# Lumina-Group/libzkp

Hardware: NVIDIA B200
Metric: groth16_bn254_proofs_per_sec_batched (higher is better)
Workload: dtype u256 (8x32-bit Montgomery limbs, integer)

## Files before the change

libzkp_b200/csrc/engine.cu:

```cuda
#include <cuda_runtime.h>
#include <atomic>
#include <cmath>
#include <cstdio>
#include <cstdlib>
#include <mutex>
#include <string>
#include <thread>
#include <type_traits>
#include <vector>

#include "common.h"
#include "host_util.h"
#include "kernels_prove.cuh"
#include "tables.h"
#include "large.h"
#include "setup.h"
#include "verify.h"

using namespace lzkp;
using namespace lzkp::eng;

static thread_local std::string g_err;
static std::mutex g_mu;
static int g_device = -1;
// ... 47 lines not shown
        CUDA_TRY(cudaMemcpyToSymbol(c_mimc, c.data(), sizeof(Fr) * 110));
        g_mimc_uploaded |= 1ull << (dev & 63);
    }
    return LZKP_OK;
}
int current_device() { return t_device >= 0 ? t_device : g_device; }
DeviceScope::DeviceScope(int dev) : prev(t_device) {
    t_device = dev;
    cudaSetDevice(dev);
}
DeviceScope::~DeviceScope() {
    t_device = prev;
    const int back = prev >= 0 ? prev : g_device;
    if (back >= 0) cudaSetDevice(back);
}
}
}


struct MsmPlan {
    DBuf table;
    DBuf unit_dig, unit_tbl;
    DBuf items[4];
    DBuf msm_items[4];
    uint32_t n_items[4] = {0, 0, 0, 0};
    uint32_t item_len[4] = {8, 32, 128, 512};
    uint32_t n_units = 0, n_rows = 0, n_msm = 0;
    std::vector<uint32_t> msm_unit_begin;
    std::vector<uint2> msm_items_host[4];
};

struct HBuf {
    void *p = nullptr;
    size_t bytes = 0;
    int ensure(size_t n) {
        if (n <= bytes) return LZKP_OK;
        if (p) cudaFreeHost(p);
        p = nullptr;
        bytes = 0;
        cudaError_t err = cudaMallocHost(&p, n);
        if (err != cudaSuccess) { p = nullptr; cudaGetLastError(); return fail(LZKP_E_NOMEM, "cudaMallocHost failed"); }
        bytes = n;
        return LZKP_OK;
    }
    template <class T> T *as() const { return reinterpret_cast<T *>(p); }
    ~HBuf() { if (p) cudaFreeHost(p); }
};
struct Workspace {
    uint32_t chunk = 0;
    DBuf z, abc, tmp, h, dig, r, s, rs, part1, part2, res1, res2, proofs, status, a, b, commit, sets, setlen, env, envlen;
    HBuf h_proofs, h_status, h_commit, h_env, h_envlen;
    cudaEvent_t last_use = nullptr;
    ~Workspace() { if (last_use) cudaEventDestroy(last_use); }
};
static int ws_acquire(Workspace &ws, cudaStream_t st) {
    if (!ws.last_use) CUDA_TRY(cudaEventCreateWithFlags(&ws.last_use, cudaEventDisableTiming));
    else CUDA_TRY(cudaStreamWaitEvent(st, ws.last_use, 0));
    return LZKP_OK;
}
static int ws_release(Workspace &ws, cudaStream_t st) {
    CUDA_TRY(cudaEventRecord(ws.last_use, st));
    return LZKP_OK;
}

struct lzkp_pk {
    std::mutex mu;
    int device = 0;
    std::vector<lzkp_pk *> replicas;
    uint32_t n_vars = 0, n_inst = 0, n_wit = 0, n = 0, log_n = 0, m = 0;
    bool has_circuit = false;
    int kind = -1;
    uint32_t kind_param = 0;
    int c = 16;
    uint32_t W = 16, N = 32768;
    uint64_t table_bytes = 0;
    uint32_t max_chunk = 8192;
    uint32_t n_dig_rows = 0, nz = 0;
    MsmPlan g1, g2;
    MsmPlan g1_lat;
    uint32_t row_sz = 0, row_rz = 0;
    bool has_lat = false;
    ProofConsts consts;
    DBuf csr_rowptr[3], csr_col[3], csr_val[3];
    CsrDev csr[3];
    DBuf tw_fwd, tw_inv, coset_br, uncoset_br;
    NttTables ntt;
    Workspace ws[2];
    bool large = false;
    bool tiled_wm = false;
    MsmBases *L_a = nullptr, *L_b1 = nullptr, *L_b2 = nullptr, *L_l = nullptr, *L_h = nullptr;
    DBuf L_sa, L_sb, L_sl, L_sb1;
    cudaStream_t L_st[3] = {nullptr, nullptr, nullptr}, L_st_scale = nullptr;
    cudaEvent_t L_ev_in = nullptr, L_ev_done[3] = {nullptr, nullptr, nullptr}, L_ev_a = nullptr, L_ev_scale = nullptr;
    uint32_t shard_index = 0, shard_count = 1, map_ranks = 1;
    bool L_scaled = false;
    uint32_t L_lo[5] = {0, 0, 0, 0, 0}, L_cnt[5] = {0, 0, 0, 0, 0};
    cudaStream_t stream = nullptr, stream2 = nullptr;
    cudaEvent_t ev_fork = nullptr, ev_join[2] = {nullptr, nullptr};
    cudaStream_t chunk_stream(int i) const { return (i & 1) ? stream2 : stream; }
    struct Mark { int region; cudaEvent_t a, b; };
    std::vector<Mark> marks;
    double prof_ms[LZKP_PROFILE_REGIONS] = {0};
    uint64_t prof_count[LZKP_PROFILE_REGIONS] = {0};
    ~lzkp_pk() {
        for (lzkp_pk *r : replicas) { DeviceScope ds(r->device); delete r; }
        for (auto &m : marks) { cudaEventDestroy(m.a); cudaEventDestroy(m.b); }
        for (MsmBases *b : {L_a, L_b1, L_b2, L_l, L_h}) if (b) msm_bases_free(b);
        for (auto s_ : L_st) if (s_) cudaStreamDestroy(s_);
        if (L_ev_in) cudaEventDestroy(L_ev_in);
        if (L_ev_a) cudaEventDestroy(L_ev_a);
        if (L_ev_scale) cudaEventDestroy(L_ev_scale);
        if (L_st_scale) cudaStreamDestroy(L_st_scale);
        for (auto ev : L_ev_done) if (ev) cudaEventDestroy(ev);
        if (ev_fork) cudaEventDestroy(ev_fork);
        for (auto ev : ev_join) if (ev) cudaEventDestroy(ev);
        if (stream2) cudaStreamDestroy(stream2);
        if (stream) cudaStreamDestroy(stream);
    }
};

struct BaseRef { uint32_t dig_row, tbl_row; };
static int finish_plan(MsmPlan &pl, const std::vector<std::vector<BaseRef>> &msms, uint32_t W) {
    std::vector<uint32_t> ud, ut;
    pl.msm_unit_begin.clear();
    for (auto &ms : msms) {
        pl.msm_unit_begin.push_back((uint32_t)ud.size());
        for (auto &b : ms)
            for (uint32_t w = 0; w < W; w++) {
                ud.push_back(b.dig_row * W + w);
                ut.push_back(b.tbl_row * W + w);
            }
    }
    pl.msm_unit_begin.push_back((uint32_t)ud.size());
    pl.n_units = (uint32_t)ud.size();
    pl.n_msm = (uint32_t)msms.size();
    TRY(upload(pl.unit_dig, ud));
    TRY(upload(pl.unit_tbl, ut));
    for (int v = 0; v < 4; v++) {
        std::vector<uint2> items, mi;
        for (uint32_t q = 0; q < pl.n_msm; q++) {
            uint32_t first = (uint32_t)items.size();
            for (uint32_t u = pl.msm_unit_begin[q]; u < pl.msm_unit_begin[q + 1]; u += pl.item_len[v])
                items.push_back(make_uint2(u, std::min(u + pl.item_len[v], pl.msm_unit_begin[q + 1])));
            mi.push_back(make_uint2(first, (uint32_t)items.size()));
        }
        pl.n_items[v] = (uint32_t)items.size();
        pl.msm_items_host[v] = mi;
        TRY(upload(pl.items[v], items));
        TRY(upload(pl.msm_items[v], mi));
    }
    return LZKP_OK;
}

static uint32_t fit_item_len(const std::vector<std::vector<BaseRef>> &msms, uint32_t W, uint32_t resident) {
    uint32_t best = 128;
    uint64_t best_cost = UINT64_MAX;
    for (uint32_t len = 96; len <= 192; len++) {
        uint64_t items = 0, cost = 0;
        for (auto &ms : msms) items += ((uint64_t)ms.size() * W + len - 1) / len;
        for (uint64_t gx : {8u, 16u, 32u, 64u}) cost += (gx * items + resident - 1) / resident * len * (64 / gx);
        if (cost < best_cost) { best_cost = cost; best = len; }
    }
    return best;
}

static inline uint32_t window_count(int c) { return (uint32_t)((255 + c - 1) / c); }

namespace {
struct Reader {
    const uint8_t *p, *end;
    bool take(size_t n, const uint8_t **out) {
        if ((size_t)(end - p) < n) return false;
        *out = p;
        p += n;
        return true;
    }
    bool g1(host::G1Canon &o) { const uint8_t *b; return take(64, &b) && host::read_g1(b, o); }
    bool g2(host::G2Canon &o) { const uint8_t *b; return take(128, &b) && host::read_g2(b, o); }
    bool vec_g1(std::vector<host::G1Canon> &v) {
        const uint8_t *b;
        if (!take(8, &b)) return false;
        uint64_t len;
        memcpy(&len, b, 8);
        if (len > (uint64_t)(end - p) / 64) return false;
        v.resize(len);
        for (auto &x : v) if (!g1(x)) return false;
        return true;
    }
    bool vec_g2(std::vector<host::G2Canon> &v) {
        const uint8_t *b;
        if (!take(8, &b)) return false;
        uint64_t len;
        memcpy(&len, b, 8);
        if (len > (uint64_t)(end - p) / 128) return false;
        v.resize(len);
        for (auto &x : v) if (!g2(x)) return false;
        return true;
    }
};
host::G1Canon neg_canon(const host::G1Canon &p) {
    host::G1Canon r = p;
    if (!host::is_inf(p)) {
        Fq m = Fq::modulus();
        sub8(r.y.l, m.l, p.y.l);
    }
    return r;
}
}

static int pk_load_impl(const uint8_t *bytes, size_t len, int validate, const lzkp_pk_options *opt, lzkp_pk *pk) {
    static_assert(sizeof(host::G1Canon) == sizeof(G1Affine) && sizeof(host::G2Canon) == sizeof(G2Affine), "layout");
    Reader rd{bytes, bytes + len};
    host::G1Canon alpha_g1, beta_g1, delta_g1;
    host::G2Canon beta_g2, gamma_g2, delta_g2;
    std::vector<host::G1Canon> gamma_abc, a_q, b1_q, h_q, l_q;
    std::vector<host::G2Canon> b2_q;
    bool ok = rd.g1(alpha_g1) && rd.g2(beta_g2) && rd.g2(gamma_g2) && rd.g2(delta_g2) && rd.vec_g1(gamma_abc) &&
              rd.g1(beta_g1) && rd.g1(delta_g1) && rd.vec_g1(a_q) && rd.vec_g1(b1_q) && rd.vec_g2(b2_q) &&
              rd.vec_g1(h_q) && rd.vec_g1(l_q);
    if (!ok || rd.p != rd.end) return fail(LZKP_E_INVALID, "proving key: malformed ark-serialize bytes");
    const uint32_t nv = (uint32_t)a_q.size();
    if (nv < 2 || b1_q.size() != nv || b2_q.size() != nv || l_q.size() >= nv || gamma_abc.size() + l_q.size() != nv)
        return fail(LZKP_E_INVALID, "proving key: inconsistent query lengths");
    const uint32_t n = (uint32_t)h_q.size() + 1;
    if (n < 2 || (n & (n - 1))) return fail(LZKP_E_INVALID, "proving key: h_query length + 1 is not a power of two");
    pk->n_vars = nv;
    pk->n_wit = (uint32_t)l_q.size();
    pk->n_inst = nv - pk->n_wit;
    pk->n = n;
    pk->log_n = 0;
    while ((1u << pk->log_n) < n) pk->log_n++;
    pk->nz = nv - 1;
    pk->n_dig_rows = pk->nz + 3 + (n - 1);
    const uint32_t ROW_R = pk->nz, ROW_S = pk->nz + 1, ROW_RS = pk->nz + 2, ROW_H = pk->nz + 3;

    {
        size_t free_b0 = 0, total_b0 = 0;
        CUDA_TRY(cudaMemGetInfo(&free_b0, &total_b0));
        const uint64_t budget0 = opt && opt->table_budget_bytes ? opt->table_budget_bytes : (uint64_t)(free_b0 * 0.6);
        const uint64_t rows1_max = 2ull * nv + pk->n_wit + n + 2, rows2_max = (uint64_t)nv + 1;
        const uint64_t min_table = (rows1_max * 64 + rows2_max * 128) * 32 * 128;
        pk->large = pk->log_n > 16 || min_table > budget0 || getenv("LZKP_FORCE_LARGE") != nullptr;
    }
    if (pk->large) {
        CUDA_TRY(cudaStreamCreate(&pk->stream));
    CUDA_TRY(cudaStreamCreate(&pk->stream2));
    CUDA_TRY(cudaEventCreateWithFlags(&pk->ev_fork, cudaEventDisableTiming));
    for (auto &ev : pk->ev_join) CUDA_TRY(cudaEventCreateWithFlags(&ev, cudaEventDisableTiming));
        const int wb = opt && opt->window_bits ? opt->window_bits : 0;
        pk->shard_count = opt && opt->shard_count > 1 ? opt->shard_count : 1;
        pk->shard_index = pk->shard_count > 1 ? opt->shard_index : 0;
        if (pk->shard_index >= pk->shard_count) return fail(LZKP_E_INVALID, "shard_index >= shard_count");
        const uint32_t G_ = pk->shard_count;
        const uint64_t w_g2 = getenv("LZKP_SHARD_G2_WEIGHT") ? (uint64_t)atoi(getenv("LZKP_SHARD_G2_WEIGHT")) : (G_ > 2 ? 32 : 28);
        const uint64_t sizes[5] = {nv, nv, (uint64_t)pk->n_wit + 1, (uint64_t)n - 1, nv}, wts[5] = {10, 10, 10, 10, w_g2};
        const double Wh = (double)sizes[3] * wts[3];
        double Wz = 0;
        for (int q : {0, 1, 2, 4}) Wz += (double)sizes[q] * wts[q];
        const double map_frac = getenv("LZKP_SHARD_MAP_COST") ? atof(getenv("LZKP_SHARD_MAP_COST")) : (G_ > 4 ? 0.085 : 0.11);
        const double M = G_ > 1 ? map_frac * (Wz + Wh) : 0.0;
        uint32_t k = 1;
        while (k < G_ && k * ((Wz + Wh + k * M) / G_ - M) < Wh) k++;
        const double T = (Wz + Wh + k * M) / G_;
        std::vector<double> cutz(G_ + 1, 0.0), share(G_, 0.0);
        for (uint32_t i = 0; i < G_; i++) share[i] = i < k ? std::max(0.0, T - M - Wh / k) : T;
        const double piece_cost = G_ > 2 ? (getenv("LZKP_SHARD_PIECE_COST") ? atof(getenv("LZKP_SHARD_PIECE_COST")) : (G_ > 4 ? 0.25 : 0.45)) * 2.76e6 : 0.0;
        std::vector<double> adj(share);
        for (int round = 0; round < 4; round++) {
            double tot = 0;
            for (uint32_t i = 0; i < G_; i++) tot += adj[i];
            for (uint32_t i = 0; i < G_; i++) cutz[i + 1] = cutz[i] + adj[i] * Wz / tot;
            double bounds[5] = {0, 0, 0, 0, 0};
            { int j = 0; for (int q : {0, 1, 2, 4}) { bounds[j + 1] = bounds[j] + (double)sizes[q] * wts[q]; j++; } }
            if (piece_cost != 0.0)
                for (uint32_t i = 1; i < G_; i++)
                    for (int j = 1; j < 4; j++)
                        if (std::fabs(cutz[i] - bounds[j]) < 1.0e5) cutz[i] = bounds[j];
            if (round == 3 || piece_cost == 0.0) break;
            double extra_total = 0;
            std::vector<double> extra(G_, 0.0);
            for (uint32_t i = 0; i < G_; i++) {
                int pieces = 0;
                for (int j = 0; j < 4; j++)
                    if (std::min(cutz[i + 1], bounds[j + 1]) - std::max(cutz[i], bounds[j]) > 1e-6 * Wz) pieces++;
                extra[i] = piece_cost * std::max(0, pieces - 1);
                extra_total += extra[i];
            }
            for (uint32_t i = 0; i < G_; i++) adj[i] = std::max(0.0, share[i] - extra[i] + extra_total / G_);
        }
        pk->map_ranks = k;
        const uint32_t me = pk->shard_index;
        if (me < k) {
            pk->L_lo[3] = (uint32_t)(sizes[3] * me / k);
            pk->L_cnt[3] = (uint32_t)(sizes[3] * (me + 1) / k) - pk->L_lo[3];
        } else {
            pk->L_lo[3] = 0;
            pk->L_cnt[3] = 0;
        }
        double acc_w = 0;
        for (int q : {0, 1, 2, 4}) {
            auto first_at = [&](double w) -> uint64_t {
                if (w <= acc_w) return 0;
                return std::min<uint64_t>((uint64_t)std::ceil((w - acc_w) / wts[q]), sizes[q]);
            };
            uint64_t lo = first_at(cutz[me]), hi = me + 1 == G_ ? sizes[q] : first_at(cutz[me + 1]);
            pk->L_lo[q] = (uint32_t)lo;
            pk->L_cnt[q] = (uint32_t)(hi - lo);
            acc_w += (double)sizes[q] * wts[q];
        }
        auto load1 = [&](std::vector<host::G1Canon> v, size_t skip, const host::G1Canon *extra, int q, MsmBases **out) {
            v.erase(v.begin(), v.begin() + skip);
            if (extra) v.push_back(*extra);
            return msm_bases_load(1, reinterpret_cast<const uint8_t *>(v.data() + pk->L_lo[q]), pk->L_cnt[q], wb, 1, validate, out, 1);
// ... 48 lines not shown
            if (bad) return fail(LZKP_E_INVALID, "proving key: " + std::to_string(bad) + " point(s) off-curve or outside the subgroup");
        }
        TRY(d_out1.alloc(2 * sizeof(G1Affine))); TRY(d_out2.alloc(sizeof(G2Affine)));
        LAUNCH((k_affine_add<Fq>), 1, 1, 0, st, d_misc1.as<G1Affine>() + 0, d_misc1.as<G1Affine>() + 2, d_out1.as<G1Affine>() + 0, 0);
        LAUNCH((k_affine_add<Fq>), 1, 1, 0, st, d_misc1.as<G1Affine>() + 1, d_misc1.as<G1Affine>() + 3, d_out1.as<G1Affine>() + 1, 0);
        LAUNCH((k_affine_add<Fq2>), 1, 1, 0, st, d_misc2.as<G2Affine>() + 0, d_misc2.as<G2Affine>() + 1, d_out2.as<G2Affine>(), 0);
        G1Affine c1[2];
        G2Affine c2;
        CUDA_TRY(cudaMemcpyAsync(c1, d_out1.p, sizeof(c1), cudaMemcpyDeviceToHost, st));
        CUDA_TRY(cudaMemcpyAsync(&c2, d_out2.p, sizeof(c2), cudaMemcpyDeviceToHost, st));
        CUDA_TRY(cudaStreamSynchronize(st));
        pk->consts.a0 = c1[0]; pk->consts.b0 = c1[1]; pk->consts.b2 = c2;
        CUDA_TRY(cudaGetLastError());
        return LZKP_OK;
    }

    std::vector<host::G1Canon> rows1;
    std::vector<host::G2Canon> rows2;
    std::vector<std::vector<BaseRef>> msm1(5), msm2(1);
    std::vector<BaseRef> a_all, b1_all;
    auto add1 = [&](const host::G1Canon &p) { rows1.push_back(p); return (uint32_t)rows1.size() - 1; };
    auto same_point = [](const host::G1Canon &u, const host::G1Canon &v) {
        return memcmp(&u.x, &v.x, sizeof(Fq)) == 0 && memcmp(&u.y, &v.y, sizeof(Fq)) == 0;
    };
    for (uint32_t j = 1; j < nv; j++) {
        const bool has_a = !host::is_inf(a_q[j]), has_b = !host::is_inf(b1_q[j]);
        if (has_a && has_b && same_point(a_q[j], b1_q[j])) {
            const BaseRef ref{j - 1, add1(a_q[j])};
            msm1[4].push_back(ref); a_all.push_back(ref); b1_all.push_back(ref);
            continue;
        }
        if (has_a) { msm1[0].push_back({j - 1, add1(a_q[j])}); a_all.push_back(msm1[0].back()); }
        if (has_b) { msm1[1].push_back({j - 1, add1(b1_q[j])}); b1_all.push_back(msm1[1].back()); }
    }
    for (uint32_t j = 0; j < pk->n_wit; j++) if (!host::is_inf(l_q[j])) msm1[2].push_back({pk->n_inst + j - 1, add1(l_q[j])});
    for (uint32_t i = 0; i + 1 < n; i++) if (!host::is_inf(h_q[i])) msm1[3].push_back({ROW_H + i, add1(h_q[i])});
    if (!host::is_inf(delta_g1)) {
        uint32_t rd1 = add1(delta_g1), rnd1 = add1(neg_canon(delta_g1));
        msm1[0].push_back({ROW_R, rd1});
        msm1[1].push_back({ROW_S, rd1});
        msm1[2].push_back({ROW_RS, rnd1});
        a_all.push_back({ROW_R, rd1});
    }
    std::vector<std::vector<BaseRef>> msm1_lat(6);
    {
        pk->row_sz = pk->n_dig_rows;
        pk->row_rz = pk->n_dig_rows + pk->nz;
        msm1_lat[0] = a_all;
        msm1_lat[2] = msm1[2];
        msm1_lat[3] = msm1[3];
        for (auto &b : a_all) if (b.dig_row < pk->nz) msm1_lat[4].push_back({pk->row_sz + b.dig_row, b.tbl_row});
        for (auto &b : b1_all) msm1_lat[5].push_back({pk->row_rz + b.dig_row, b.tbl_row});
        auto mont = [](const host::G1Canon &c) { return G1Affine{Fq::from_canonical(c.x), Fq::from_canonical(c.y)}; };
        auto canon = [](const G1Affine &m) { host::G1Canon c; c.x = m.x.to_canonical(); c.y = m.y.to_canonical(); return c; };
        auto sum2 = [&](const host::G1Canon &u, const host::G1Canon &v) {
            G1XYZZ t = host::is_inf(u) ? G1XYZZ::inf() : G1XYZZ::from_affine(mont(u));
            if (!host::is_inf(v)) t.madd(mont(v));
            return t.is_inf() ? host::G1Canon{Fq::zero(), Fq::zero()} : canon(t.to_affine());
        };
        const host::G1Canon a0c = sum2(alpha_g1, a_q[0]), b0c = sum2(beta_g1, b1_q[0]), d2c = sum2(delta_g1, delta_g1);
        if (!host::is_inf(a0c)) msm1_lat[4].push_back({ROW_S, add1(a0c)});
        if (!host::is_inf(b0c)) msm1_lat[5].push_back({ROW_R, add1(b0c)});
        if (!host::is_inf(d2c)) msm1_lat[5].push_back({ROW_RS, add1(d2c)});
        pk->n_dig_rows += 2 * pk->nz;
        pk->has_lat = true;
    }
    for (uint32_t j = 1; j < nv; j++)
        if (!host::is_inf(b2_q[j])) { rows2.push_back(b2_q[j]); msm2[0].push_back({j - 1, (uint32_t)rows2.size() - 1}); }
    if (!host::is_inf(delta_g2)) { rows2.push_back(delta_g2); msm2[0].push_back({ROW_S, (uint32_t)rows2.size() - 1}); }
    pk->g1.n_rows = (uint32_t)rows1.size();
    pk->g2.n_rows = (uint32_t)rows2.size();

    size_t free_b = 0, total_b = 0;
    CUDA_TRY(cudaMemGetInfo(&free_b, &total_b));
    uint64_t budget = opt && opt->table_budget_bytes ? opt->table_budget_bytes : (uint64_t)(free_b * 0.6);
    int c = opt && opt->window_bits ? opt->window_bits : 0;
    if (const char *e = getenv("LZKP_WINDOW_BITS")) if (!c) c = atoi(e);
    auto bytes_for = [&](int cc) {
        uint64_t W = window_count(cc), N = 1ull << (cc - 1);
        return (rows1.size() * 64ull + rows2.size() * 128ull) * W * N;
    };
    if (c == 0) {
        c = 16;
        while (c > 8 && bytes_for(c) > budget) c--;
    }
    if (c < 8 || c > 17) return fail(LZKP_E_INVALID, "window_bits must be in [8,17]");
    if (bytes_for(c) > free_b) return fail(LZKP_E_NOMEM, "window tables do not fit in device memory");
    pk->c = c;
    pk->W = window_count(c);
    pk->N = 1u << (c - 1);
    pk->table_bytes = bytes_for(c);
    pk->max_chunk = opt && opt->max_chunk ? opt->max_chunk : 8192;
    if (pk->max_chunk > 32768) pk->max_chunk = 32768;

    CUDA_TRY(cudaStreamCreate(&pk->stream));
    CUDA_TRY(cudaStreamCreate(&pk->stream2));
    CUDA_TRY(cudaEventCreateWithFlags(&pk->ev_fork, cudaEventDisableTiming));
    for (auto &ev : pk->ev_join) CUDA_TRY(cudaEventCreateWithFlags(&ev, cudaEventDisableTiming));
    CUDA_TRY(cudaStreamCreateWithFlags(&pk->L_st[0], cudaStreamNonBlocking));
    CUDA_TRY(cudaEventCreateWithFlags(&pk->L_ev_in, cudaEventDisableTiming));
    CUDA_TRY(cudaEventCreateWithFlags(&pk->L_ev_done[0], cudaEventDisableTiming));
    cudaStream_t st = pk->stream;

    std::vector<host::G1Canon> misc1 = {alpha_g1, beta_g1, delta_g1, a_q[0], b1_q[0]};
    std::vector<host::G2Canon> misc2 = {beta_g2, gamma_g2, delta_g2, b2_q[0]};
    DBuf d_rows1, d_rows2, d_misc1, d_misc2, d_out1, d_out2;
    TRY(upload(d_rows1, rows1)); TRY(upload(d_rows2, rows2)); TRY(upload(d_misc1, misc1)); TRY(upload(d_misc2, misc2));
    auto to_mont = [&](DBuf &b, size_t n_fq) {
        if (n_fq) LAUNCH(k_fq_to_mont, (unsigned)((n_fq + 127) / 128), 128, 0, st, b.as<Fq>(), n_fq);
    };
    to_mont(d_rows1, rows1.size() * 2); to_mont(d_rows2, rows2.size() * 4);
    to_mont(d_misc1, misc1.size() * 2); to_mont(d_misc2, misc2.size() * 4);
    if (validate) {
        std::vector<host::G1Canon> all1 = gamma_abc;
        std::vector<host::G2Canon> all2;
        DBuf d_all1, d_bad;
        TRY(upload(d_all1, all1));
        to_mont(d_all1, all1.size() * 2);
        TRY(d_bad.alloc(sizeof(int)));
        CUDA_TRY(cudaMemsetAsync(d_bad.p, 0, sizeof(int), st));
        auto chk1 = [&](DBuf &b, size_t cnt) {
            if (cnt) LAUNCH(k_check_g1, (unsigned)((cnt + 63) / 64), 64, 0, st, b.as<G1Affine>(), (uint32_t)cnt, d_bad.as<int>());
        };
        auto chk2 = [&](DBuf &b, size_t cnt) {
            if (cnt) LAUNCH(k_check_g2, (unsigned)((cnt + 63) / 64), 64, 0, st, b.as<G2Affine>(), (uint32_t)cnt, d_bad.as<int>());
        };
        chk1(d_rows1, rows1.size()); chk1(d_misc1, misc1.size()); chk1(d_all1, all1.size());
        chk2(d_rows2, rows2.size()); chk2(d_misc2, misc2.size());
        int bad = 0;
        CUDA_TRY(cudaMemcpyAsync(&bad, d_bad.p, sizeof(int), cudaMemcpyDeviceToHost, st));
        CUDA_TRY(cudaStreamSynchronize(st));
        if (bad) return fail(LZKP_E_INVALID, "proving key: " + std::to_string(bad) + " point(s) off-curve or outside the subgroup");
    }
    TRY(d_out1.alloc(2 * sizeof(G1Affine))); TRY(d_out2.alloc(sizeof(G2Affine)));
    LAUNCH((k_affine_add<Fq>), 1, 1, 0, st, d_misc1.as<G1Affine>() + 0, d_misc1.as<G1Affine>() + 3, d_out1.as<G1Affine>() + 0, 0);
    LAUNCH((k_affine_add<Fq>), 1, 1, 0, st, d_misc1.as<G1Affine>() + 1, d_misc1.as<G1Affine>() + 4, d_out1.as<G1Affine>() + 1, 0);
    LAUNCH((k_affine_add<Fq2>), 1, 1, 0, st, d_misc2.as<G2Affine>() + 0, d_misc2.as<G2Affine>() + 3, d_out2.as<G2Affine>(), 0);
    G1Affine c1[2];
    G2Affine c2;
    CUDA_TRY(cudaMemcpyAsync(c1, d_out1.p, sizeof(c1), cudaMemcpyDeviceToHost, st));
    CUDA_TRY(cudaMemcpyAsync(&c2, d_out2.p, sizeof(c2), cudaMemcpyDeviceToHost, st));
    CUDA_TRY(cudaStreamSynchronize(st));
    pk->consts.a0 = c1[0]; pk->consts.b0 = c1[1]; pk->consts.b2 = c2;

    TRY(pk->g1.table.alloc((size_t)rows1.size() * pk->W * pk->N * sizeof(G1Affine)));
    TRY(pk->g2.table.alloc((size_t)rows2.size() * pk->W * pk->N * sizeof(G2Affine)));
    if (!rows1.empty())
        TRY(build_table_g1(d_rows1.p, (uint32_t)rows1.size(), c, pk->W, pk->N, pk->g1.table.p, st));
    if (!rows2.empty())
        TRY(build_table_g2(d_rows2.p, (uint32_t)rows2.size(), c, pk->W, pk->N, pk->g2.table.p, st));
    {
        uint32_t resident = 0;
        TRY(batch_msm_g1_resident(c > 16 ? 4 : 2, &resident));
        pk->g1.item_len[2] = fit_item_len(msm1, pk->W, resident);
    }
    TRY(finish_plan(pk->g1, msm1, pk->W));
    TRY(finish_plan(pk->g1_lat, msm1_lat, pk->W));
    TRY(finish_plan(pk->g2, msm2, pk->W));
    {
        const uint64_t per_proof = (uint64_t)nv * 32 + 7ull * n * 32 + (uint64_t)pk->n_dig_rows * pk->W * (c > 16 ? 4 : 2) +
                                   (uint64_t)pk->g1.n_items[2] * sizeof(G1XYZZ) + (uint64_t)pk->g2.n_items[1] * sizeof(G2XYZZ) +
                                   4 * sizeof(G1XYZZ) + sizeof(G2XYZZ) + 1024;
        size_t free_now = 0, total_now = 0;
        CUDA_TRY(cudaMemGetInfo(&free_now, &total_now));
        uint64_t fit = (uint64_t)(free_now * 0.4) / (2 * per_proof);
        fit = std::max<uint64_t>(32, fit / 32 * 32);
        if (pk->max_chunk > fit) pk->max_chunk = (uint32_t)fit;
    }
    CUDA_TRY(cudaGetLastError());
    return LZKP_OK;
}

static int circuit_install(lzkp_pk *pk, uint32_t m, uint32_t n_inst, uint32_t n_wit, const uint32_t *const rowptr[3],
                           const uint32_t *const col[3], const uint8_t *const val[3]) {
    if (n_inst != pk->n_inst || n_wit != pk->n_wit) return fail(LZKP_E_INVALID, "circuit shape does not match the proving key");
    uint64_t need = (uint64_t)m + n_inst;
    uint32_t n = 1;
    while (n < need) n <<= 1;
    if (n != pk->n) return fail(LZKP_E_INVALID, "circuit domain size does not match the proving key's h_query");
    pk->tiled_wm = pk->large || pk->log_n > 12;
    cudaStream_t st = pk->stream;
    for (int k = 0; k < 3; k++) {
        uint32_t nnz = rowptr[k][m];
        for (uint32_t i = 0; i < nnz; i++) if (col[k][i] >= pk->n_vars) return fail(LZKP_E_INVALID, "matrix column out of range");
        TRY(pk->csr_rowptr[k].alloc(sizeof(uint32_t) * (m + 1)));
        TRY(pk->csr_col[k].alloc(sizeof(uint32_t) * nnz));
        TRY(pk->csr_val[k].alloc(sizeof(Fr) * (size_t)nnz));
        CUDA_TRY(cudaMemcpy(pk->csr_rowptr[k].p, rowptr[k], sizeof(uint32_t) * (m + 1), cudaMemcpyHostToDevice));
        if (nnz) {
            CUDA_TRY(cudaMemcpy(pk->csr_col[k].p, col[k], sizeof(uint32_t) * nnz, cudaMemcpyHostToDevice));
            CUDA_TRY(cudaMemcpy(pk->csr_val[k].p, val[k], 32 * (size_t)nnz, cudaMemcpyHostToDevice));
            LAUNCH(k_to_r2_form, (nnz + 127) / 128, 128, 0, st, pk->csr_val[k].as<Fr>(), nnz);
        }
        pk->csr[k] = CsrDev{pk->csr_rowptr[k].as<uint32_t>(), pk->csr_col[k].as<uint32_t>(), pk->csr_val[k].as<Fr>()};
    }
    pk->m = m;
    Fr w, wi, g, gi;
    for (int i = 0; i < 8; i++) { w.l[i] = FrParams::ROOT28(i); wi.l[i] = FrParams::ROOT28_INV(i); g.l[i] = FrParams::GEN(i); gi.l[i] = FrParams::GEN_INV(i); }
    for (uint32_t i = pk->log_n; i < 28; i++) { w = w.sqr(); wi = wi.sqr(); }
    Fr ninv = host::fr_from_u64(n).inverse();
    Fr gn = g;
    for (uint32_t i = 0; i < pk->log_n; i++) gn = gn.sqr();
    Fr zinv = (gn - Fr::one()).inverse();
    if (pk->tiled_wm) {
        pk->ntt = NttTables{nullptr, nullptr, nullptr, nullptr, nullptr, ninv, zinv};
        CUDA_TRY(cudaStreamSynchronize(st));
        CUDA_TRY(cudaGetLastError());
        pk->has_circuit = true;
        return LZKP_OK;
    }
    TRY(pk->tw_fwd.alloc(sizeof(Fr) * (n / 2))); TRY(pk->tw_inv.alloc(sizeof(Fr) * (n / 2)));
    TRY(pk->coset_br.alloc(sizeof(Fr) * n)); TRY(pk->uncoset_br.alloc(sizeof(Fr) * n));
    LAUNCH(k_pow_table, (n / 2 + 127) / 128, 128, 0, st, pk->tw_fwd.as<Fr>(), w, Fr::one(), n / 2, 0u);
    LAUNCH(k_pow_table, (n / 2 + 127) / 128, 128, 0, st, pk->tw_inv.as<Fr>(), wi, Fr::one(), n / 2, 0u);
    LAUNCH(k_pow_table, (n + 127) / 128, 128, 0, st, pk->coset_br.as<Fr>(), g, ninv, n, pk->log_n);
    LAUNCH(k_pow_table, (n + 127) / 128, 128, 0, st, pk->uncoset_br.as<Fr>(), gi, ninv.to_canonical(), n, pk->log_n);
    pk->ntt = NttTables{pk->tw_fwd.as<Fr>(), pk->tw_inv.as<Fr>(), pk->coset_br.as<Fr>(), pk->uncoset_br.as<Fr>(), nullptr, ninv, zinv};
    size_t smem = (size_t)32 * n;
    if (smem > 48 * 1024) {
        CUDA_TRY(cudaFuncSetAttribute(k_ntt_icoset, cudaFuncAttributeMaxDynamicSharedMemorySize, (int)smem));
        CUDA_TRY(cudaFuncSetAttribute(k_ntt_final, cudaFuncAttributeMaxDynamicSharedMemorySize, (int)smem));
    }
    CUDA_TRY(cudaStreamSynchronize(st));
    CUDA_TRY(cudaGetLastError());
    pk->has_circuit = true;
    return LZKP_OK;
}

static inline int item_variant(uint32_t P) {
    return P > small_batch_limit() ? (P >= 256 ? 2 : 1) : 0;
}
static inline int fit_variant(const MsmPlan &pl, int v) {
    while (v < 3 && pl.n_items[v] > 65535u) v++;
    return v;
}
static inline uint32_t latency_limit() {
    static const uint32_t v = getenv("LZKP_LATENCY_BATCH") ? (uint32_t)atoi(getenv("LZKP_LATENCY_BATCH")) : 384u;
    return v;
}
static inline bool use_lat(const lzkp_pk *pk, uint32_t P) { return pk->has_lat && P <= latency_limit() && P <= small_batch_limit(); }
static inline int item_variant_g2(uint32_t P) {
    return P > small_batch_limit() ? 1 : 0;
}
static int ensure_workspace(lzkp_pk *pk, Workspace &ws, uint32_t P) {
    if (P <= ws.chunk) return LZKP_OK;
    size_t part1 = 0, part2 = 0;
    for (uint32_t pp : {std::min(P, small_batch_limit()), std::min(P, std::max(latency_limit(), 1u)), std::min(P, 255u), std::min(P, 2047u), P}) {
        part1 = std::max(part1, (size_t)pk->g1.n_items[fit_variant(pk->g1, item_variant(pp))] * pp);
        if (use_lat(pk, pp)) part1 = std::max(part1, (size_t)pk->g1_lat.n_items[fit_variant(pk->g1_lat, item_variant(pp))] * pp);
        part2 = std::max(part2, (size_t)pk->g2.n_items[fit_variant(pk->g2, item_variant_g2(pp))] * pp);
    }
    const size_t nv = pk->n_vars, n = pk->n;
    TRY(ws.z.ensure(P * nv * 32));
    TRY(ws.abc.ensure(3 * P * n * 32));
    TRY(ws.h.ensure(P * n * 32));
    if (pk->tiled_wm) TRY(ws.tmp.ensure(3 * P * n * 32));
    if (pk->large) {
        TRY(pk->L_sa.ensure(nv * 32)); TRY(pk->L_sb.ensure(nv * 32)); TRY(pk->L_sb1.ensure(nv * 32)); TRY(pk->L_sl.ensure(((size_t)pk->n_wit + 1) * 32));
    } else {
        TRY(ws.dig.ensure((size_t)pk->n_dig_rows * pk->W * P * (pk->c > 16 ? 4 : 2)));
    }
    TRY(ws.r.ensure(P * 32)); TRY(ws.s.ensure(P * 32)); TRY(ws.rs.ensure(P * 32));
    TRY(ws.part1.ensure(part1 * sizeof(G1XYZZ)));
    TRY(ws.part2.ensure(part2 * sizeof(G2XYZZ)));
    TRY(ws.res1.ensure((size_t)6 * P * sizeof(G1XYZZ)));
    TRY(ws.res2.ensure((size_t)P * sizeof(G2XYZZ)));
    TRY(ws.proofs.ensure((size_t)P * 256));
    TRY(ws.status.ensure((size_t)P * sizeof(int32_t)));
    TRY(ws.a.ensure(P * 8)); TRY(ws.b.ensure(P * 8)); TRY(ws.commit.ensure(P * 32));
    ws.chunk = P;
    return LZKP_OK;
}

static inline void wires_to_canonical(Fr *z, uint32_t P, uint32_t nv, uint32_t first, uint32_t count, cudaStream_t st) {
    const size_t total = (size_t)P * count;
    LAUNCH(k_wires_to_canonical, (unsigned)((total + 127) / 128), 128, 0, st, z, P, nv, first, count);
}

struct Region {
    lzkp_pk *pk;
    cudaStream_t st;
    cudaEvent_t b = nullptr;
    Region(lzkp_pk *pk_, int region, cudaStream_t st_) : pk(pk_), st(st_) {
        if (!g_profile.load(std::memory_order_relaxed) || pk->marks.size() > 65536) return;
        cudaEvent_t a;
        if (cudaEventCreate(&a) != cudaSuccess || cudaEventCreate(&b) != cudaSuccess) { b = nullptr; return; }
        cudaEventRecord(a, st);
        pk->marks.push_back({region, a, b});
    }
    ~Region() { if (b) cudaEventRecord(b, st); }
};

static int run_witness_map(lzkp_pk *pk, Workspace &ws, uint32_t P, cudaStream_t st) {
    const uint32_t n = pk->n, threads = std::max(32u, std::min(n / 2, 512u));
    const size_t smem = (size_t)32 * n;
    Region reg(pk, LZKP_REGION_WITNESS_MAP, st);
    if (pk->tiled_wm) {
        Fr *abc = ws.abc.as<Fr>(), *tmp = ws.tmp.as<Fr>(), *h = ws.h.as<Fr>();
        const size_t plane = (size_t)P * n;
        LAUNCH(k_spmv_abc, dim3((n + 127) / 128, P), 128, 0, st, pk->csr[0], pk->csr[1], pk->csr[2], ws.z.as<Fr>(), abc, P,
               pk->n_vars, pk->m, pk->n_inst, n);
        TRY(large_ntt_device(abc, tmp, pk->log_n, 1, 0, st, 3 * P, n));
        TRY(large_ntt_device(tmp, abc, pk->log_n, 0, 1, st, 3 * P, n));
        LAUNCH(k_pointwise_h, (unsigned)((plane + 127) / 128), 128, 0, st, abc, abc + plane, abc + 2 * plane, tmp, pk->ntt.zinv,
               plane);
        TRY(large_ntt_device(tmp, h, pk->log_n, 1, 1, st, P, n));
        LAUNCH(k_fr_to_canonical, (unsigned)((plane + 127) / 128), 128, 0, st, h, plane);
// ... 924 lines not shown
```

libzkp_b200/csrc/msm_batch.cu:

```cuda
#include <algorithm>
#include <cstdlib>
#include "tables.h"
#include "dev_util.cuh"

#ifndef LZKP_G2_MINB
#define LZKP_G2_MINB 6
#endif
#ifndef LZKP_G1_MINB
#define LZKP_G1_MINB 4
#endif
#define LZKP_G2_MINB_SEL(F) (sizeof(F) == sizeof(::lzkp::Fq) ? LZKP_G1_MINB : LZKP_G2_MINB)
namespace lzkp {

template <class F, int BLOCK, class DigT>
__global__ void __launch_bounds__(BLOCK, LZKP_G2_MINB_SEL(F)) k_msm_batch(const Affine<F> *__restrict__ table, uint32_t N,
                                                     const uint32_t *__restrict__ unit_dig,
                                                     const uint32_t *__restrict__ unit_tbl,
                                                     const uint2 *__restrict__ items, const DigT *__restrict__ dig,
                                                     uint32_t P, XYZZ<F> *__restrict__ partial) {
    const uint32_t p = blockIdx.x * BLOCK + threadIdx.x, item = blockIdx.y;
    if (p >= P) return;
    const uint2 range = items[item];
    XYZZ<F> acc = XYZZ<F>::inf();
    int d = dig[(size_t)__ldg(unit_dig + range.x) * P + p];
    Affine<F> pt = Affine<F>::inf();
    if (d) pt = gather_point(table, N, __ldg(unit_tbl + range.x), d);
    for (uint32_t u = range.x; u < range.y; u++) {
        int dn = 0;
        Affine<F> ptn = Affine<F>::inf();
        if (u + 1 < range.y) {
            dn = dig[(size_t)__ldg(unit_dig + u + 1) * P + p];
            if (dn) ptn = gather_point(table, N, __ldg(unit_tbl + u + 1), dn);
        }
        if (d) acc.madd(pt);
        d = dn;
        pt = ptn;
    }
    st_vec(partial + (size_t)item * P + p, acc);
}
template <class F>
__global__ void __launch_bounds__(128) k_msm_reduce1(XYZZ<F> *partial, const uint2 *msm_items, uint32_t P, uint32_t G) {
    uint32_t p = blockIdx.x * blockDim.x + threadIdx.x, q = blockIdx.y, g = blockIdx.z;
    if (p >= P) return;
    uint2 r = msm_items[q];
    if (r.x + g >= r.y) return;
    XYZZ<F> acc = ld_vec(partial + (size_t)(r.x + g) * P + p);
    for (uint32_t it = r.x + g + G; it < r.y; it += G) acc.add_cold(ld_vec(partial + (size_t)it * P + p));
    st_vec(partial + (size_t)(r.x + g) * P + p, acc);
}
template <class F>
__global__ void __launch_bounds__(128) k_msm_reduce(const XYZZ<F> *partial, const uint2 *msm_items, uint32_t P,
                                                    uint32_t G, XYZZ<F> *out) {
    uint32_t p = blockIdx.x * blockDim.x + threadIdx.x, q = blockIdx.y;
    if (p >= P) return;
    uint2 r = msm_items[q];
    uint32_t end = min(r.y, r.x + G);
    XYZZ<F> acc = XYZZ<F>::inf();
    for (uint32_t it = r.x; it < end; it++) acc.add_cold(ld_vec(partial + (size_t)it * P + p));
    st_vec(out + (size_t)q * P + p, acc);
}

template <class F>
__global__ void __launch_bounds__(128) k_msm_fold(XYZZ<F> *partial, const uint2 *msm_items, uint32_t P, uint32_t half,
                                                  XYZZ<F> *out) {
    uint32_t p = blockIdx.x * blockDim.x + threadIdx.x, q = blockIdx.y, g = blockIdx.z;
    if (p >= P) return;
    const uint2 r = msm_items[q];
    const uint32_t live = min(r.y - r.x, 2 * half);
    if (g >= live) {
        if (half == 1 && g == 0) st_vec(out + (size_t)q * P + p, XYZZ<F>::inf());
        return;
    }
    XYZZ<F> acc = ld_vec(partial + (size_t)(r.x + g) * P + p);
    if (g + half < live) acc.add_cold(ld_vec(partial + (size_t)(r.x + g + half) * P + p));
    if (half == 1) st_vec(out + (size_t)q * P + p, acc);
    else st_vec(partial + (size_t)(r.x + g) * P + p, acc);
}

template <class F, int T>
__global__ void __launch_bounds__(T) k_msm_reduce_tree(const XYZZ<F> *__restrict__ partial, const uint2 *__restrict__ msm_items,
                                                       uint32_t P, XYZZ<F> *__restrict__ out) {
    __shared__ uint4 raw[T * sizeof(XYZZ<F>) / 16];
    XYZZ<F> *sm = reinterpret_cast<XYZZ<F> *>(raw);
    const uint32_t p = blockIdx.x, q = blockIdx.y, t = threadIdx.x;
    const uint2 r = msm_items[q];
    XYZZ<F> acc = XYZZ<F>::inf();
    for (uint32_t it = r.x + t; it < r.y; it += T) acc.add_cold(ld_vec(partial + (size_t)it * P + p));
    st_vec(sm + t, acc);
    __syncthreads();
    for (uint32_t s = T / 2; s > 0; s >>= 1) {
        if (t < s) {
            XYZZ<F> a = ld_vec(sm + t);
            a.add_cold(ld_vec(sm + t + s));
            st_vec(sm + t, a);
        }
        __syncthreads();
    }
    if (t == 0) st_vec(out + (size_t)q * P + p, ld_vec(sm));
}

}

namespace lzkp {
namespace eng {
uint32_t small_batch_limit() {
    static const uint32_t v = [] {
        const char *e = getenv("LZKP_SMALL_BATCH");
        return e ? (uint32_t)atoi(e) : 512u;
    }();
    return v;
}

int batch_msm_g1_resident(uint32_t dig_bytes, uint32_t *out) {
    int dev = 0, sms = 0, per_sm = 0;
    CUDA_TRY(cudaGetDevice(&dev));
    CUDA_TRY(cudaDeviceGetAttribute(&sms, cudaDevAttrMultiProcessorCount, dev));
    if (dig_bytes == 2) CUDA_TRY(cudaOccupancyMaxActiveBlocksPerMultiprocessor(&per_sm, k_msm_batch<Fq, 128, int16_t>, 128, 0));
    else CUDA_TRY(cudaOccupancyMaxActiveBlocksPerMultiprocessor(&per_sm, k_msm_batch<Fq, 128, int32_t>, 128, 0));
    *out = (uint32_t)std::max(1, sms * per_sm);
    return LZKP_OK;
}

void batch_msm_g1_items(const BatchMsmArgs &a, uint32_t item0, uint32_t count, cudaStream_t st) {
    if (!count) return;
    if (a.P <= small_batch_limit()) {
        if (a.dig_bytes == 2)
            LAUNCH((k_msm_batch<Fq, 32, int16_t>), dim3((a.P + 31) / 32, count), 32, 0, st, (const G1Affine *)a.table, a.N, a.unit_dig, a.unit_tbl,
                   (const uint2 *)a.items + item0, (const int16_t *)a.dig, a.P, (G1XYZZ *)a.partial + (size_t)item0 * a.P);
        else
            LAUNCH((k_msm_batch<Fq, 32, int32_t>), dim3((a.P + 31) / 32, count), 32, 0, st, (const G1Affine *)a.table, a.N, a.unit_dig, a.unit_tbl,
                   (const uint2 *)a.items + item0, (const int32_t *)a.dig, a.P, (G1XYZZ *)a.partial + (size_t)item0 * a.P);
        return;
    }
    if (a.dig_bytes == 2)
        LAUNCH((k_msm_batch<Fq, 128, int16_t>), dim3((a.P + 127) / 128, count), 128, 0, st, (const G1Affine *)a.table, a.N, a.unit_dig,
               a.unit_tbl, (const uint2 *)a.items + item0, (const int16_t *)a.dig, a.P, (G1XYZZ *)a.partial + (size_t)item0 * a.P);
    else
        LAUNCH((k_msm_batch<Fq, 128, int32_t>), dim3((a.P + 127) / 128, count), 128, 0, st, (const G1Affine *)a.table, a.N, a.unit_dig,
               a.unit_tbl, (const uint2 *)a.items + item0, (const int32_t *)a.dig, a.P, (G1XYZZ *)a.partial + (size_t)item0 * a.P);
}
constexpr uint32_t kReduceFan = 8;
void batch_msm_g1_reduce(const BatchMsmArgs &a, cudaStream_t st) {
    if (a.P <= small_batch_limit()) {
        LAUNCH((k_msm_reduce_tree<Fq, 128>), dim3(a.P, a.n_msm), 128, 0, st, (const G1XYZZ *)a.partial, (const uint2 *)a.msm_items,
               a.P, (G1XYZZ *)a.out);
        return;
    }
    LAUNCH((k_msm_reduce1<Fq>), dim3((a.P + 127) / 128, a.n_msm, kReduceFan), 128, 0, st, (G1XYZZ *)a.partial,
           (const uint2 *)a.msm_items, a.P, kReduceFan);
    for (uint32_t half = kReduceFan / 2; half >= 1; half >>= 1)
        LAUNCH((k_msm_fold<Fq>), dim3((a.P + 127) / 128, a.n_msm, half), 128, 0, st, (G1XYZZ *)a.partial,
               (const uint2 *)a.msm_items, a.P, half, (G1XYZZ *)a.out);
}
void batch_msm_g1(const BatchMsmArgs &a, cudaStream_t st) {
    batch_msm_g1_items(a, 0, a.n_items, st);
    batch_msm_g1_reduce(a, st);
}
void batch_msm_g2(const BatchMsmArgs &a, cudaStream_t st) {
    if (a.P <= small_batch_limit()) {
        if (a.dig_bytes == 2)
            LAUNCH((k_msm_batch<Fq2, 32, int16_t>), dim3((a.P + 31) / 32, a.n_items), 32, 0, st, (const G2Affine *)a.table, a.N, a.unit_dig,
                   a.unit_tbl, (const uint2 *)a.items, (const int16_t *)a.dig, a.P, (G2XYZZ *)a.partial);
        else
            LAUNCH((k_msm_batch<Fq2, 32, int32_t>), dim3((a.P + 31) / 32, a.n_items), 32, 0, st, (const G2Affine *)a.table, a.N, a.unit_dig,
                   a.unit_tbl, (const uint2 *)a.items, (const int32_t *)a.dig, a.P, (G2XYZZ *)a.partial);
        LAUNCH((k_msm_reduce_tree<Fq2, 128>), dim3(a.P, a.n_msm), 128, 0, st, (const G2XYZZ *)a.partial, (const uint2 *)a.msm_items,
               a.P, (G2XYZZ *)a.out);
        return;
    }
    if (a.dig_bytes == 2)
        LAUNCH((k_msm_batch<Fq2, 64, int16_t>), dim3((a.P + 63) / 64, a.n_items), 64, 0, st, (const G2Affine *)a.table, a.N,
               a.unit_dig, a.unit_tbl, (const uint2 *)a.items, (const int16_t *)a.dig, a.P, (G2XYZZ *)a.partial);
    else
        LAUNCH((k_msm_batch<Fq2, 64, int32_t>), dim3((a.P + 63) / 64, a.n_items), 64, 0, st, (const G2Affine *)a.table, a.N,
               a.unit_dig, a.unit_tbl, (const uint2 *)a.items, (const int32_t *)a.dig, a.P, (G2XYZZ *)a.partial);
    LAUNCH((k_msm_reduce1<Fq2>), dim3((a.P + 127) / 128, a.n_msm, 2 * kReduceFan), 128, 0, st, (G2XYZZ *)a.partial,
           (const uint2 *)a.msm_items, a.P, 2 * kReduceFan);
    for (uint32_t half = kReduceFan; half >= 1; half >>= 1)
        LAUNCH((k_msm_fold<Fq2>), dim3((a.P + 127) / 128, a.n_msm, half), 128, 0, st, (G2XYZZ *)a.partial,
               (const uint2 *)a.msm_items, a.P, half, (G2XYZZ *)a.out);
}

}
}
```

libzkp_b200/csrc/tables.h:

```cpp
#pragma once
#include "common.h"

namespace lzkp {
namespace eng {

int build_table_g1(const void *d_bases, uint32_t rows, int c, uint32_t W, uint32_t N, void *d_table, cudaStream_t st);
int build_table_g2(const void *d_bases, uint32_t rows, int c, uint32_t W, uint32_t N, void *d_table, cudaStream_t st);

struct BatchMsmArgs {
    const void *table;
    uint32_t N;
    const uint32_t *unit_dig, *unit_tbl;
    const void *items;
    uint32_t n_items;
    const void *msm_items;
    uint32_t n_msm;
    const void *dig;
    uint32_t dig_bytes;
    uint32_t P;
    void *partial;
    void *out;
};
void batch_msm_g1(const BatchMsmArgs &a, cudaStream_t st);
void batch_msm_g1_items(const BatchMsmArgs &a, uint32_t item0, uint32_t count, cudaStream_t st);
void batch_msm_g1_reduce(const BatchMsmArgs &a, cudaStream_t st);
void batch_msm_g2(const BatchMsmArgs &a, cudaStream_t st);
int batch_msm_g1_resident(uint32_t dig_bytes, uint32_t *out);
uint32_t small_batch_limit();

}
}
```

Before: 178,500.

## Stage G2 batch MSM points through cp.async shared-memory ring with smem accumulator

Replaces the large-batch G2 MSM kernel with one that prefetches table points into a double-buffered shared-memory ring via cp.async, and keeps the XYZZ accumulator and temporaries in shared memory to relieve register pressure. The G2 item length is now tuned with an occupancy-aware cost model, and the G1 cost model is generalized to batch sizes and block width. This adds heavy shared-memory traffic per field op and a fixed per-block smem footprint that may cap occupancy. Note that digits are read past the range end and return zero, so correctness relies on that guard.

```diff
diff --git a/libzkp_b200/csrc/engine.cu b/libzkp_b200/csrc/engine.cu
--- a/libzkp_b200/csrc/engine.cu
+++ b/libzkp_b200/csrc/engine.cu
@@ -223,13 +223,14 @@
     return LZKP_OK;
 }
 
-static uint32_t fit_item_len(const std::vector<std::vector<BaseRef>> &msms, uint32_t W, uint32_t resident) {
-    uint32_t best = 128;
+static uint32_t fit_item_len(const std::vector<std::vector<BaseRef>> &msms, uint32_t W, uint32_t resident, uint32_t block,
+                             uint32_t lo, uint32_t hi) {
+    uint32_t best = lo;
     uint64_t best_cost = UINT64_MAX;
-    for (uint32_t len = 96; len <= 192; len++) {
+    for (uint32_t len = lo; len <= hi; len++) {
         uint64_t items = 0, cost = 0;
         for (auto &ms : msms) items += ((uint64_t)ms.size() * W + len - 1) / len;
-        for (uint64_t gx : {8u, 16u, 32u, 64u}) cost += (gx * items + resident - 1) / resident * len * (64 / gx);
+        for (uint64_t P : {1024u, 2048u, 4096u, 8192u}) cost += (P / block * items + resident - 1) / resident * len * (8192 / P);
         if (cost < best_cost) { best_cost = cost; best = len; }
     }
     return best;
@@ -584,7 +585,9 @@
     {
         uint32_t resident = 0;
         TRY(batch_msm_g1_resident(c > 16 ? 4 : 2, &resident));
-        pk->g1.item_len[2] = fit_item_len(msm1, pk->W, resident);
+        pk->g1.item_len[2] = fit_item_len(msm1, pk->W, resident, 128, 96, 192);
+        TRY(batch_msm_g2_resident(c > 16 ? 4 : 2, &resident));
+        pk->g2.item_len[1] = fit_item_len(msm2, pk->W, resident, 64, 24, 64);
     }
     TRY(finish_plan(pk->g1, msm1, pk->W));
     TRY(finish_plan(pk->g1_lat, msm1_lat, pk->W));
diff --git a/libzkp_b200/csrc/msm_batch.cu b/libzkp_b200/csrc/msm_batch.cu
--- a/libzkp_b200/csrc/msm_batch.cu
+++ b/libzkp_b200/csrc/msm_batch.cu
@@ -37,6 +37,109 @@
         pt = ptn;
     }
     st_vec(partial + (size_t)item * P + p, acc);
+}
+
+constexpr int kG2Block = 64, kG2Depth = 2;
+__device__ __forceinline__ void cp_async16(void *smem, const void *gmem) {
+    asm volatile("cp.async.cg.shared.global [%0], [%1], 16;" ::"r"((uint32_t)__cvta_generic_to_shared(smem)), "l"(gmem)
+                 : "memory");
+}
+__device__ __forceinline__ void cp_async_commit() { asm volatile("cp.async.commit_group;" ::: "memory"); }
+template <int N>
+__device__ __forceinline__ void cp_async_wait() { asm volatile("cp.async.wait_group %0;" ::"n"(N) : "memory"); }
+
+__device__ __forceinline__ Fq2 lds_fq2(uint32_t addr) {
+    Fq2 r;
+    uint32_t *w = reinterpret_cast<uint32_t *>(&r);
+#pragma unroll
+    for (int i = 0; i < 4; i++)
+        asm volatile("ld.shared.v4.u32 {%0, %1, %2, %3}, [%4];"
+                     : "=r"(w[4 * i]), "=r"(w[4 * i + 1]), "=r"(w[4 * i + 2]), "=r"(w[4 * i + 3])
+                     : "r"(addr + i * kG2Block * 16)
+                     : "memory");
+    return r;
+}
+__device__ __forceinline__ void sts_fq2(uint32_t addr, const Fq2 &v) {
+    const uint32_t *w = reinterpret_cast<const uint32_t *>(&v);
+#pragma unroll
+    for (int i = 0; i < 4; i++)
+        asm volatile("st.shared.v4.u32 [%0], {%1, %2, %3, %4};" ::"r"(addr + i * kG2Block * 16), "r"(w[4 * i]),
+                     "r"(w[4 * i + 1]), "r"(w[4 * i + 2]), "r"(w[4 * i + 3])
+                     : "memory");
+}
+constexpr uint32_t kG2Field = 4 * kG2Block * 16;
+__device__ __forceinline__ void g2_store_acc(uint32_t acc, const G2XYZZ &v) {
+    sts_fq2(acc, v.x); sts_fq2(acc + kG2Field, v.y); sts_fq2(acc + 2 * kG2Field, v.zz); sts_fq2(acc + 3 * kG2Field, v.zzz);
+}
+__device__ __forceinline__ void g2_madd_staged(uint32_t acc, uint32_t pt, bool neg) {
+    const uint32_t ax = acc, ay = acc + kG2Field, azz = acc + 2 * kG2Field, azzz = acc + 3 * kG2Field;
+    if (lds_fq2(azz).is_zero()) {
+        const Fq2 y = lds_fq2(pt + kG2Field);
+        g2_store_acc(acc, G2XYZZ{lds_fq2(pt), neg ? y.neg() : y, Fq2::one(), Fq2::one()});
+        return;
+    }
+    const Fq2 U2 = lds_fq2(pt) * lds_fq2(azz);
+    Fq2 S2 = lds_fq2(pt + kG2Field) * lds_fq2(azzz);
+    if (neg) S2 = S2.neg();
+    const Fq2 Pp = U2 - lds_fq2(ax), R = S2 - lds_fq2(ay);
+    if (Pp.is_zero()) {
+        if (R.is_zero()) {
+            const Fq2 y = lds_fq2(pt + kG2Field);
+            g2_store_acc(acc, G2XYZZ::dbl_affine(G2Affine{lds_fq2(pt), neg ? y.neg() : y}));
+        } else {
+            g2_store_acc(acc, G2XYZZ::inf());
+        }
+        return;
+    }
+    const uint32_t sR = acc + 4 * kG2Field, sPPP = pt, sQ = pt + kG2Field;
+    sts_fq2(sR, R);
+    const Fq2 PP = Pp.sqr();
+    sts_fq2(sPPP, Pp * PP);
+    sts_fq2(sQ, lds_fq2(ax) * PP);
+    sts_fq2(azz, lds_fq2(azz) * PP);
+    const Fq2 X3 = lds_fq2(sR).sqr() - lds_fq2(sPPP) - lds_fq2(sQ).dbl();
+    sts_fq2(ax, X3);
+    const Fq2 RT = lds_fq2(sR) * (lds_fq2(sQ) - X3);
+    sts_fq2(ay, RT - lds_fq2(ay) * lds_fq2(sPPP));
+    sts_fq2(azzz, lds_fq2(azzz) * lds_fq2(sPPP));
+}
+template <class DigT>
+__global__ void __launch_bounds__(kG2Block, LZKP_G2_MINB) k_msm_g2_staged(const G2Affine *__restrict__ table, uint32_t N,
+                                                                        const uint32_t *__restrict__ unit_dig,
+                                                                        const uint32_t *__restrict__ unit_tbl,
+                                                                        const uint2 *__restrict__ items,
+                                                                        const DigT *__restrict__ dig, uint32_t P,
+                                                                        G2XYZZ *__restrict__ partial) {
+    __shared__ uint4 acc_s[5][4][kG2Block];
+    __shared__ uint4 ring[kG2Depth][2][4][kG2Block];
+    const uint32_t t = threadIdx.x, p = blockIdx.x * kG2Block + t, item = blockIdx.y;
+    if (p >= P) return;
+    const uint2 range = items[item];
+    const uint32_t acc = (uint32_t)__cvta_generic_to_shared(&acc_s[0][0][t]);
+    auto digit = [&](uint32_t u) { return u < range.y ? (int)dig[(size_t)__ldg(unit_dig + u) * P + p] : 0; };
+    auto stage = [&](uint32_t u, int d, int slot) {
+        if (d) {
+            const uint4 *src = reinterpret_cast<const uint4 *>(table + (size_t)__ldg(unit_tbl + u) * N + (uint32_t)(abs(d) - 1));
+#pragma unroll
+            for (int i = 0; i < 8; i++) cp_async16(&ring[slot][i / 4][i % 4][t], src + i);
+        }
+        cp_async_commit();
+    };
+    g2_store_acc(acc, G2XYZZ::inf());
+    int d0 = digit(range.x), d1 = digit(range.x + 1);
+    stage(range.x, d0, 0);
+    int slot = 0;
+    for (uint32_t u = range.x; u < range.y; u++) {
+        const int d2 = digit(u + 2);
+        stage(u + 1, d1, slot ^ 1);
+        cp_async_wait<kG2Depth - 1>();
+        if (d0) g2_madd_staged(acc, (uint32_t)__cvta_generic_to_shared(&ring[slot][0][0][t]), d0 < 0);
+        d0 = d1; d1 = d2;
+        slot ^= 1;
+    }
+    cp_async_wait<0>();
+    const G2XYZZ r{lds_fq2(acc), lds_fq2(acc + kG2Field), lds_fq2(acc + 2 * kG2Field), lds_fq2(acc + 3 * kG2Field)};
+    st_vec(partial + (size_t)item * P + p, r);
 }
 template <class F>
 __global__ void __launch_bounds__(128) k_msm_reduce1(XYZZ<F> *partial, const uint2 *msm_items, uint32_t P, uint32_t G) {
@@ -121,6 +224,16 @@
     return LZKP_OK;
 }
 
+int batch_msm_g2_resident(uint32_t dig_bytes, uint32_t *out) {
+    int dev = 0, sms = 0, per_sm = 0;
+    CUDA_TRY(cudaGetDevice(&dev));
+    CUDA_TRY(cudaDeviceGetAttribute(&sms, cudaDevAttrMultiProcessorCount, dev));
+    if (dig_bytes == 2) CUDA_TRY(cudaOccupancyMaxActiveBlocksPerMultiprocessor(&per_sm, k_msm_g2_staged<int16_t>, kG2Block, 0));
+    else CUDA_TRY(cudaOccupancyMaxActiveBlocksPerMultiprocessor(&per_sm, k_msm_g2_staged<int32_t>, kG2Block, 0));
+    *out = (uint32_t)std::max(1, sms * per_sm);
+    return LZKP_OK;
+}
+
 void batch_msm_g1_items(const BatchMsmArgs &a, uint32_t item0, uint32_t count, cudaStream_t st) {
     if (!count) return;
     if (a.P <= small_batch_limit()) {
@@ -168,12 +281,13 @@
                a.P, (G2XYZZ *)a.out);
         return;
     }
+    const dim3 grid((a.P + kG2Block - 1) / kG2Block, a.n_items);
     if (a.dig_bytes == 2)
-        LAUNCH((k_msm_batch<Fq2, 64, int16_t>), dim3((a.P + 63) / 64, a.n_items), 64, 0, st, (const G2Affine *)a.table, a.N,
-               a.unit_dig, a.unit_tbl, (const uint2 *)a.items, (const int16_t *)a.dig, a.P, (G2XYZZ *)a.partial);
+        LAUNCH((k_msm_g2_staged<int16_t>), grid, kG2Block, 0, st, (const G2Affine *)a.table, a.N, a.unit_dig, a.unit_tbl,
+               (const uint2 *)a.items, (const int16_t *)a.dig, a.P, (G2XYZZ *)a.partial);
     else
-        LAUNCH((k_msm_batch<Fq2, 64, int32_t>), dim3((a.P + 63) / 64, a.n_items), 64, 0, st, (const G2Affine *)a.table, a.N,
-               a.unit_dig, a.unit_tbl, (const uint2 *)a.items, (const int32_t *)a.dig, a.P, (G2XYZZ *)a.partial);
+        LAUNCH((k_msm_g2_staged<int32_t>), grid, kG2Block, 0, st, (const G2Affine *)a.table, a.N, a.unit_dig, a.unit_tbl,
+               (const uint2 *)a.items, (const int32_t *)a.dig, a.P, (G2XYZZ *)a.partial);
     LAUNCH((k_msm_reduce1<Fq2>), dim3((a.P + 127) / 128, a.n_msm, 2 * kReduceFan), 128, 0, st, (G2XYZZ *)a.partial,
            (const uint2 *)a.msm_items, a.P, 2 * kReduceFan);
     for (uint32_t half = kReduceFan; half >= 1; half >>= 1)
diff --git a/libzkp_b200/csrc/tables.h b/libzkp_b200/csrc/tables.h
--- a/libzkp_b200/csrc/tables.h
+++ b/libzkp_b200/csrc/tables.h
@@ -26,6 +26,7 @@
 void batch_msm_g1_reduce(const BatchMsmArgs &a, cudaStream_t st);
 void batch_msm_g2(const BatchMsmArgs &a, cudaStream_t st);
 int batch_msm_g1_resident(uint32_t dig_bytes, uint32_t *out);
+int batch_msm_g2_resident(uint32_t dig_bytes, uint32_t *out);
 uint32_t small_batch_limit();
 
 }
```

After: 181,700, median of 6. +1.8%, better.

## Pipeline MSM point gathers and digit loads through shared memory with cp.async

Applied to the files above, without the earlier changes.

Replaces the register-based one-ahead prefetch in the batched MSM kernel with a multi-stage cp.async pipeline. Table points for upcoming units are copied into shared memory several iterations ahead, and digits are staged in double-buffered chunks. The goal is to hide global gather latency behind the madd arithmetic. In exchange it uses a large amount of shared memory per block, especially for G2 points, which can lower occupancy. The 16-bit digit path, which uses an odd/even mask, adds complexity and correctness risk.

```diff
diff --git a/libzkp_b200/csrc/msm_batch.cu b/libzkp_b200/csrc/msm_batch.cu
--- a/libzkp_b200/csrc/msm_batch.cu
+++ b/libzkp_b200/csrc/msm_batch.cu
@@ -10,7 +10,25 @@
 #define LZKP_G1_MINB 4
 #endif
 #define LZKP_G2_MINB_SEL(F) (sizeof(F) == sizeof(::lzkp::Fq) ? LZKP_G1_MINB : LZKP_G2_MINB)
+#ifndef LZKP_GATHER_STAGES
+#define LZKP_GATHER_STAGES 3
+#endif
+#ifndef LZKP_DIGIT_CHUNK
+#define LZKP_DIGIT_CHUNK 16
+#endif
 namespace lzkp {
+
+__device__ __forceinline__ void cp_async16(void *smem, const void *gmem) {
+    asm volatile("cp.async.cg.shared.global [%0], [%1], 16;\n" ::"r"((uint32_t)__cvta_generic_to_shared(smem)), "l"(gmem)
+                 : "memory");
+}
+__device__ __forceinline__ void cp_async4(void *smem, const void *gmem) {
+    asm volatile("cp.async.ca.shared.global [%0], [%1], 4;\n" ::"r"((uint32_t)__cvta_generic_to_shared(smem)), "l"(gmem)
+                 : "memory");
+}
+__device__ __forceinline__ void cp_async_commit() { asm volatile("cp.async.commit_group;\n" ::: "memory"); }
+template <int N>
+__device__ __forceinline__ void cp_async_wait() { asm volatile("cp.async.wait_group %0;\n" ::"n"(N) : "memory"); }
 
 template <class F, int BLOCK, class DigT>
 __global__ void __launch_bounds__(BLOCK, LZKP_G2_MINB_SEL(F)) k_msm_batch(const Affine<F> *__restrict__ table, uint32_t N,
@@ -18,23 +36,69 @@
                                                      const uint32_t *__restrict__ unit_tbl,
                                                      const uint2 *__restrict__ items, const DigT *__restrict__ dig,
                                                      uint32_t P, XYZZ<F> *__restrict__ partial) {
-    const uint32_t p = blockIdx.x * BLOCK + threadIdx.x, item = blockIdx.y;
+    constexpr int S = LZKP_GATHER_STAGES, DC = LZKP_DIGIT_CHUNK, NV = sizeof(Affine<F>) / 16;
+    static_assert(S >= 2 && DC >= 2 * S - 1 && DC <= 32, "digit chunk k+1 must land before unit (k+1)*DC is gathered");
+    __shared__ uint4 s_pt[S][NV][BLOCK];
+    __shared__ uint32_t s_dig[2][DC][BLOCK];
+    const uint32_t t = threadIdx.x, p = blockIdx.x * BLOCK + t, item = blockIdx.y;
     if (p >= P) return;
     const uint2 range = items[item];
+    const uint32_t L = range.y - range.x;
+    uint32_t odd0 = 0, odd1 = 0;
+    auto copy_digits = [&](uint32_t k) {
+        const uint32_t b = k & 1, u0 = k * DC;
+        uint32_t o = 0;
+#pragma unroll
+        for (int j = 0; j < DC; j++) {
+            if (u0 + j < L) {
+                const size_t idx = (size_t)__ldg(unit_dig + range.x + u0 + j) * P + p;
+                if constexpr (sizeof(DigT) == 4) {
+                    cp_async4(&s_dig[b][j][t], dig + idx);
+                } else {
+                    o |= (uint32_t)(idx & 1) << j;
+                    cp_async4(&s_dig[b][j][t], dig + (idx & ~(size_t)1));
+                }
+            }
+        }
+        if (b) odd1 = o; else odd0 = o;
+    };
+    auto digit = [&](uint32_t u) -> int {
+        const uint32_t b = (u / DC) & 1, j = u % DC, w = s_dig[b][j][t];
+        if constexpr (sizeof(DigT) == 4) return (int)w;
+        else return (int)(int16_t)(w >> (16 * (((b ? odd1 : odd0) >> j) & 1)));
+    };
+    auto gather = [&](uint32_t u) {
+        const int d = digit(u);
+        if (!d) return;
+        const uint4 *src = reinterpret_cast<const uint4 *>(table + (size_t)__ldg(unit_tbl + range.x + u) * N + (uint32_t)(abs(d) - 1));
+#pragma unroll
+        for (int v = 0; v < NV; v++) cp_async16(&s_pt[u % S][v][t], src + v);
+    };
+
+    copy_digits(0);
+    cp_async_commit();
+    cp_async_wait<0>();
+#pragma unroll
+    for (int j = 0; j < S - 1; j++) {
+        if ((uint32_t)j < L) gather(j);
+        cp_async_commit();
+    }
     XYZZ<F> acc = XYZZ<F>::inf();
-    int d = dig[(size_t)__ldg(unit_dig + range.x) * P + p];
-    Affine<F> pt = Affine<F>::inf();
-    if (d) pt = gather_point(table, N, __ldg(unit_tbl + range.x), d);
-    for (uint32_t u = range.x; u < range.y; u++) {
-        int dn = 0;
-        Affine<F> ptn = Affine<F>::inf();
-        if (u + 1 < range.y) {
-            dn = dig[(size_t)__ldg(unit_dig + u + 1) * P + p];
-            if (dn) ptn = gather_point(table, N, __ldg(unit_tbl + u + 1), dn);
+#pragma unroll 1
+    for (uint32_t i = 0; i < L; i++) {
+        if (i + S - 1 < L) gather(i + S - 1);
+        if (i % DC == 0 && i + DC < L) copy_digits(i / DC + 1);
+        cp_async_commit();
+        cp_async_wait<S - 1>();
+        const int d = digit(i);
+        if (d) {
+            Affine<F> pt;
+            uint4 *v = reinterpret_cast<uint4 *>(&pt);
+#pragma unroll
+            for (int k = 0; k < NV; k++) v[k] = s_pt[i % S][k][t];
+            if (d < 0) pt.y = pt.y.neg();
+            acc.madd(pt);
         }
-        if (d) acc.madd(pt);
-        d = dn;
-        pt = ptn;
     }
     st_vec(partial + (size_t)item * P + p, acc);
 }
```

New measurement: 178,500 before, 182,300 after (median of 6 runs). 2.1% higher.
